# ucsdarclab/Python-SuPer

Measured on AMD Instinct MI355X. Metric: LM iterations/s (embedded-deformation LM, point-to-plane + ARAP + Rot), higher is better.
Workload: dtype f64; 1 GPU; C2: 200000 surfels / 2000 ED nodes / KNN=4, point-to-plane + ARAP + Rot, 10 LM iterations + Surfels.update per frame; frames_per_gpu=8, streams_per_gpu=1, global_frames=8, parallelism=frames sharded over 1 GPU(s), beta all-gather

## Files before the change

include/super_lm.h:

```cpp
#ifndef SUPER_LM_H
#define SUPER_LM_H

#include <stdint.h>

#ifdef __cplusplus
extern "C" {
#endif

enum {
  SLM_OK = 0,
  SLM_ERR_INVALID = 1,
  SLM_ERR_HIP = 2,
  SLM_ERR_NO_DEVICE = 3,
  SLM_ERR_UNBOUND = 4,
  SLM_ERR_UNSUPPORTED = 5
};

enum {
  SLM_ITER_OK = 0,
  SLM_ITER_SOLVER_FAILED = 1,
  SLM_ITER_NOT_RUN = 2,
  SLM_ITER_SOLVER_TIMEOUT = 3
};

// ... 342 lines not shown

typedef struct slm_graph_outputs {
  int32_t cap_nodes, pad;
  double* points;
  double* norms;
  double* radii;
  int32_t* edge_index;
  double* edges_lens;
  int32_t* triangles;
  double* triangles_areas;
} slm_graph_outputs;

int slm_graph_init(int32_t H, int32_t W, int32_t step, const uint8_t* valid, const int32_t* index_map,
                   const double* points, const double* norms, const slm_graph_outputs* out,
                   int32_t* counts_host, void* stream);

int slm_graph_init_semantic(int32_t H, int32_t W, int32_t step, const uint8_t* valid, const int32_t* index_map,
                            const double* points, const double* norms, int32_t num_classes, const double* seg_conf,
                            int32_t prune_class_edges, const slm_graph_outputs* out, int32_t* node_seg,
                            double* node_seg_conf, int32_t* counts_host, void* stream);

int slm_debug_last_solver_form(slm_solver* s);
int slm_debug_last_dag_mode(slm_solver* s);
int slm_debug_counters(int64_t out[4]);
int slm_debug_dag_trace(slm_solver* s, int32_t slot, int32_t on, void* stream);
int slm_debug_dag_timeout(int64_t ticks);
int slm_debug_dag_abort(slm_solver* s, int32_t n_frames, void* stream);
int slm_debug_read(slm_solver* s, int32_t slot, int32_t what, double* host_out, int64_t max_doubles,
                   int64_t* n_doubles, void* stream);
int slm_debug_read_plan(slm_solver* s, int32_t slot, int32_t what, void* host_out, int64_t max_bytes, int64_t* n_bytes,
                        void* stream);

#ifdef __cplusplus
}
#endif
#endif
```

python-super_amd/csrc/slm_api.hip:

```cpp
#include <atomic>
#include <condition_variable>
#include <functional>
#include <mutex>
#include <new>
#include <string>
#include <thread>
#include <algorithm>
#include <vector>
#include <cstdio>
#include <cstring>

#include "slm_common.h"
#include "slm_prep.h"

void launch_data_grad(const FrameDev*, int, int, int, double, hipStream_t);
void launch_data_grad_pairs(const FrameDev*, int, int, int, double, hipStream_t);
void launch_data_loss(const FrameDev*, int, int, int, double, int, hipStream_t);
void launch_data_resid(const FrameDev*, int, int, int, double, double*, uint8_t*, int32_t*, hipStream_t);
void launch_data_gram(const FrameDev*, int, int, double, int, hipStream_t, const int* reuse = nullptr);
void launch_begin_and_gram(const FrameDev*, int, int, double, hipStream_t, const int* reuse, int dag_cut);
void launch_data_eval(const FrameDev*, int, int, double, int mode, hipStream_t, const int* reuse = nullptr);
void launch_band_assemble(const FrameDev*, int, int, hipStream_t);
void launch_reg_grad(const FrameDev*, int, int, int, double, int, double, hipStream_t);
void launch_front_assemble(const FrameDev*, int, int, hipStream_t);
void launch_pair_reduce(const FrameDev*, int, int, hipStream_t);
void launch_pair_scatter(const FrameDev*, int, int, hipStream_t);
void launch_reg_grad_nd(const FrameDev*, int, int, int, double, int, double, hipStream_t);
void launch_front_load_rhs(const FrameDev*, int, int, hipStream_t);
void launch_iter_begin_nd(const FrameDev*, int, hipStream_t, const int* reuse, int dag_cut);
void launch_front_solve(const FrameDev*, int, const NDLevelSched*, int, double, hipStream_t);
int launch_front_solve_dag(const FrameDev*, int, int, double, hipStream_t, int cut, bool reset, bool check);
int dag_device_setup(int dev, int* xcd8_out);
int dag_last_mode();
void launch_after_solve(const FrameDev*, int, int, int, int, double, int, double, int, hipStream_t);
hipError_t set_dag_timeout_ticks(long long);
void launch_dag_abort_check(const FrameDev*, int, hipStream_t);
void launch_front_levels(const FrameDev*, int, const NDLevelSched*, int, int, int, double, hipStream_t);
void launch_reg_loss(const FrameDev*, int, int, int, double, int, double, int, hipStream_t);
void launch_bandwidth(const slm_frame&, int*, hipStream_t);
void launch_band_solve(const FrameDev*, int, int, int, double, hipStream_t);
void launch_band_to_dense(const FrameDev*, int, double*, hipStream_t);
void launch_dense_to_band(const FrameDev*, const double*, const double*, hipStream_t);
void launch_init_slot(const FrameDev*, int, int, const slm_config&, hipStream_t);
void launch_iter_begin(const FrameDev*, int, hipStream_t);
void launch_pack_nodes(const FrameDev*, int, int, hipStream_t);
void launch_make_trial(const FrameDev*, int, int, hipStream_t);
void launch_pack_target(int, const float*, const float*, float4*, hipStream_t);
void launch_pack_target_px(int, const int*, const uint8_t*, const float*, const float*, float4*, hipStream_t);
void launch_accept(const FrameDev*, int, int, int, int, hipStream_t, int* reuse = nullptr, int eval_pass = 0);
void launch_loss_out(const FrameDev*, int, int, double*, hipStream_t);
void launch_zero_reg_part(const FrameDev*, int, int, hipStream_t);
void launch_update(int, int, int, float*, float*, const int*, const float*, float*, float*, const double*,
                   hipStream_t);
void launch_update64(int, int, int, double*, double*, const int*, const double*, double*, double*, const double*,
                     hipStream_t);
void launch_knn(int, int, int, int, const float*, const float*, int*, float*, hipStream_t);
void launch_knn64(int, int, int, int, const double*, const double*, const int*, const int*, int*, double*, int*,
                  hipStream_t);
void launch_knn_weights64(int, int, int, const int*, const double*, const double*, int, const double*, const double*,
                          double*, uint8_t*, hipStream_t);
// ... 220 lines not shown
  std::vector<std::thread> threads_;
  std::mutex m_;
  std::condition_variable cv_work_, cv_done_;
  const std::function<void(int)>* job_ = nullptr;
  int generation_ = 0, n_active_ = 0, pending_ = 0;
  bool stop_ = false;
};
}

struct slm_solver {
  PrepBuffers* prep = nullptr;
  BindPool bind_pool;
  AsyncWorker prep_worker;
  PrepBuffers* prep_async = nullptr;
  hipStream_t prep_stream = nullptr;
  std::vector<PrepBuffers*> bind_prep;
  std::vector<hipStream_t> bind_streams;
  std::vector<hipEvent_t> bind_events;
  std::mutex band_mutex;
  hipEvent_t drain_event = nullptr;
  double drain_est_ms = 0.0;
  int last_solver_form = -1;
  int last_dag_mode = -1;
  bool no_reuse = false;
  bool hybrid_batches = true;
  long dag_max_nodes = 8000;
  bool fuse_begin = true;
  bool pure_fill = true;
  bool profile = false;
  std::vector<hipEvent_t> ev_pool;
  std::vector<std::vector<hipEvent_t>> ev_runs;
  slm_config cfg{};
  std::vector<Slot> slots;
  FrameDev* frames_dev = nullptr;
  int* bw_dev = nullptr;
  int* bw_host = nullptr;
  int* reuse_dev = nullptr;
  int rank = 0, world = 1;
  bool shard_mode = false;
};
namespace {
bool solve_is_task_graph(const slm_solver* s, int n, int J);
}

static std::atomic<long long> g_reallocs{0}, g_realloc_bytes{0}, g_plan_builds{0}, g_plan_reuses{0}, g_plan_fill_hits{0};

// ... 9 lines not shown
  }
  size_t want = need + need / 8;
  hipError_t e = hipMalloc((void**)&p, want * sizeof(T));
  if (e == hipSuccess) cap = want;
  return e;
}
template <typename T>
static hipError_t grow(GP<T>& p, size_t& cap, size_t need) {
  T* q = p;
  const hipError_t e = grow(q, cap, need);
  p = q;
  return e;
}

static int check_slots(slm_solver* s, int first, int n);
static int check_slots_fwd(slm_solver* s, int first, int n) { return check_slots(s, first, n); }

extern "C" {

const char* slm_last_error(void) { return g_err.c_str(); }

int slm_debug_last_solver_form(slm_solver* s) { return s ? s->last_solver_form : -1; }
int slm_debug_last_dag_mode(slm_solver* s) { return s ? s->last_dag_mode : -1; }

int slm_debug_counters(int64_t out[4]) {
  if (!out) return fail(SLM_ERR_INVALID, "slm_debug_counters: null output");
  out[0] = g_reallocs;
  out[1] = g_realloc_bytes;
  out[2] = g_plan_builds;
  out[3] = g_plan_reuses;
  return SLM_OK;
}

int slm_debug_dag_timeout(int64_t ticks) {
  if (ticks < 0) return fail(SLM_ERR_INVALID, "slm_debug_dag_timeout: negative");
  HIPCHK(set_dag_timeout_ticks(ticks == 0 ? 300000000ll : (long long)ticks));
  return SLM_OK;
}

int slm_debug_dag_abort(slm_solver* s, int32_t n_frames, void* stream) {
  int rc = check_slots_fwd(s, 0, n_frames);
  if (rc) return rc;
  for (int i = 0; i < n_frames; ++i)
    if (!s->slots[i].h.nd_ready) return fail(SLM_ERR_UNSUPPORTED, "slm_debug_dag_abort: every slot needs a nested-dissection plan");
  hipStream_t st = (hipStream_t)stream;
  launch_dag_abort_check(s->frames_dev, n_frames, st);
// ... 114 lines not shown
  } catch (...) {
    delete s;
    return fail(SLM_ERR_HIP, "slm_create: out of host memory");
  }
  hipError_t e = hipMalloc((void**)&s->frames_dev, sizeof(FrameDev) * cfg->max_frames);
  if (e == hipSuccess) e = hipMemset(s->frames_dev, 0, sizeof(FrameDev) * cfg->max_frames);
  if (e == hipSuccess) e = hipMalloc((void**)&s->bw_dev, 2 * sizeof(int));
  if (e == hipSuccess) e = hipMalloc((void**)&s->reuse_dev, sizeof(int) * cfg->max_frames);
  if (e == hipSuccess) e = hipMemset(s->reuse_dev, 0, sizeof(int) * cfg->max_frames);
  if (e == hipSuccess) e = hipHostMalloc((void**)&s->bw_host, 2 * sizeof(int), hipHostMallocDefault);
  if (e == hipSuccess) {
    s->prep = prep_create();
    if (!s->prep) e = hipErrorOutOfMemory;
  }
  if (e != hipSuccess) {
    g_err = std::string("slm_create: ") + hipGetErrorString(e);
    slm_destroy(s);
    return SLM_ERR_HIP;
  }
  {
    int dev = 0;
    (void)hipGetDevice(&dev);
    (void)dag_device_setup(dev, nullptr);
  }
  if (const char* hb = getenv("SLM_HYBRID")) s->hybrid_batches = atoi(hb) != 0;
  if (const char* dm = getenv("SLM_DAG_MAX_NODES")) s->dag_max_nodes = atol(dm);
  if (const char* nr = getenv("SLM_NO_REUSE")) s->no_reuse = atoi(nr) != 0;
  if (const char* pf = getenv("SLM_PURE_FILL")) s->pure_fill = atoi(pf) != 0;
  if (const char* fb = getenv("SLM_FUSE_BEGIN")) s->fuse_begin = atoi(fb) != 0;
  *out = s;
  return SLM_OK;
}

int slm_destroy(slm_solver* s) {
  if (!s) return SLM_OK;
  s->prep_worker.shutdown();
  s->bind_pool.shutdown();
  for (Slot& sl : s->slots) {
    FrameDev& h = sl.h;
    if (h.beta) (void)hipFree(h.beta);
    if (h.delta) (void)hipFree(h.delta);
    if (h.rhs) (void)hipFree(h.rhs);
    if (sl.band) (void)hipFree(sl.band);
    if (sl.linv) (void)hipFree(sl.linv);
    if (h.loss_part) (void)hipFree(h.loss_part);
    if (h.st) (void)hipFree(h.st);
    if (h.rec) (void)hipFree(h.rec);
// ... 764 lines not shown
  if (s->cfg.use_arap || s->cfg.use_rot)
    d.n_reg_part = std::min(kRegBlocksMax, (d.maxJKe + 255) / 256);
  return d;
}

static bool solve_is_task_graph(const slm_solver* s, int n, int J) {
  return s->cfg.solver_path == 2 || (s->cfg.solver_path == 0 && (n <= 2 || (long)n * J <= s->dag_max_nodes));
}
static bool solve_is_hybrid(const slm_solver* s, int n, const BatchDims& d) {
  return !solve_is_task_graph(s, n, d.maxP / 7) && (s->cfg.solver_path == 4 || (s->cfg.solver_path == 0 && s->hybrid_batches)) &&
         d.hybrid_cut >= 0 && d.hybrid_levels == (int)d.sched.size() && d.hybrid_cut + 1 < d.hybrid_levels;
}
static int dag_cut_of(const slm_solver* s, int n, const BatchDims& d) {
  if (solve_is_task_graph(s, n, d.maxP / 7)) return -1;
  return solve_is_hybrid(s, n, d) ? d.hybrid_cut : -2;
}
int enqueue_front_solve(slm_solver* s, const FrameDev* fr, int n, const BatchDims& d, double u_override, hipStream_t st,
                        bool dag_reset_done = false, bool dag_check_later = false) {
  const bool dag = solve_is_task_graph(s, n, d.maxP / 7);
  const bool hybrid = solve_is_hybrid(s, n, d);
  s->last_solver_form = dag ? 1 : (hybrid ? 2 : 0);
  int mode = -1;
  if (dag) {
    mode = launch_front_solve_dag(fr, n, d.max_tasks, u_override, st, -1, !dag_reset_done, !dag_check_later);
  } else if (hybrid) {
    const int n_levels = (int)d.sched.size(), l_cut = n_levels - 1 - d.hybrid_cut;
    launch_front_levels(fr, n, d.sched.data(), n_levels, l_cut, 0, u_override, st);
    mode = launch_front_solve_dag(fr, n, d.max_top_tasks, u_override, st, d.hybrid_cut, !dag_reset_done, !dag_check_later);
  } else {
    launch_front_solve(fr, n, d.sched.data(), (int)d.sched.size(), u_override, st);
  }
  s->last_dag_mode = mode;
  return mode;
}

int enqueue_assemble_nd(slm_solver* s, int first, int n, const BatchDims& d, hipStream_t st) {
  const FrameDev* fr = s->frames_dev + first;
  if (s->cfg.use_data && !d.v1 && !d.vk)
    return fail(SLM_ERR_UNSUPPORTED, "slm_solve: a multifrontal slot without a multifrontal data path");
  launch_iter_begin_nd(fr, n, st, nullptr, -2);
  if (s->cfg.use_data) {
    if (d.v1) {
      launch_data_eval(fr, n, kLossBlocks, s->cfg.w_data, 2, st);
      launch_data_gram(fr, n, d.max_pos, s->cfg.w_data, d.gram_variants, st);
      launch_front_assemble(fr, n, d.max_blocks, st);
    } else {
      launch_data_grad_pairs(fr, n, d.maxN, d.K, s->cfg.w_data, st);
      launch_pair_scatter(fr, n, d.max_blocks, st);
    }
  }
  launch_reg_grad_nd(fr, n, d.maxP / 7, s->cfg.use_arap, s->cfg.w_arap, s->cfg.use_rot, s->cfg.w_rot, st);
  if (!s->cfg.use_arap && !s->cfg.use_rot) launch_front_load_rhs(fr, n, d.maxP, st);
  return SLM_OK;
// ... 579 lines not shown
```

python-super_amd/csrc/slm_front.hip:

```cpp
#include <algorithm>
#include <atomic>
#include <cstdlib>

#include "slm_tile.h"
#include "slm_begin.h"

__device__ __forceinline__ int nd_base(const NDFront& f, int p) {
  return p < f.nv ? 7 * p : f.n1p + 7 * (p - f.nv);
}

__device__ __forceinline__ double* ftile(const FrameDev& fd, const NDFront& f, int r, int c) {
  const size_t t = (size_t)c * f.nt - (size_t)c * (c - 1) / 2 + (size_t)(r - c);
  return fd.ftiles + f.tile_off + t * TILE;
}

__device__ __forceinline__ double* front_entry(const FrameDev& fd, const NDFront& f, int i, int j) {
  return ftile(fd, f, i >> 6, j >> 6) + (i & 63) + (size_t)(j & 63) * NB;
}

__device__ __forceinline__ double* dest_entry(const FrameDev& fd, const NDDest& d, int x, int y) {
  const NDFront& f = fd.fronts[d.front];
  const int rb = nd_base(f, d.prow), cb = nd_base(f, d.pcol);
  return d.transpose ? front_entry(fd, f, rb + y, cb + x) : front_entry(fd, f, rb + x, cb + y);
}
// ... 667 lines not shown
    }
    __syncthreads();
    for (int sc = c + 1; sc < f.npt; ++sc) {
      const double* Ls = ftile(fd, f, sc, c);
      double breg[16];
#pragma unroll
      for (int e = 0; e < 16; ++e) breg[e] = Ls[threadIdx.x + 256 * e];
      __syncthreads();
#pragma unroll
      for (int e = 0; e < 16; ++e) Bl[threadIdx.x + 256 * e] = breg[e];
      __syncthreads();
      for (int r = sc; r < f.npt; ++r) {
        double* Ct = ftile(fd, f, r, sc);
        double areg[16];
        load_a_frags(ftile(fd, f, r, c), areg);
        double4_t acc[4];
        load_c_frags(Ct, acc);
        if (r == sc) tile_ABt_regs_trim<true>(areg, Bl, acc, 4, w + 1);
        else tile_ABt_regs<true>(areg, Bl, acc);
        store_c_frags(Ct, acc);
      }
    }
    __syncthreads();
  }
}

__global__ void __launch_bounds__(256, 3) k_fL21(const FrameDev* __restrict__ frames, LevelRef lvl, WgMap map) {
  __shared__ double Bl[TILE];
  __shared__ double yv[NB];
  WgId wg;
  if (!wg_decode(map, wg)) return;
  const FrameDev& fd = frames[wg.frame];
  if (!fd.bound || !fd.nd_ready) return;
  int fi;
  if (!level_front(fd, lvl, wg.front, fi)) return;
  const NDFront& f = fd.fronts[fi];
  const int r = f.npt + wg.unit;
  if (f.npt == 0 || r >= f.nt) return;
  const int w = threadIdx.x >> 6, l = threadIdx.x & 63, lr = l & 15, lk = l >> 4;
  double* vecs = fd.fvec + f.vec_off;
  const bool wave_on = 16 * w < min(NB, 7 * f.nb - NB * wg.unit);
  double rhs_acc = 0.0;
  for (int c = 0; c < f.npt; ++c) {
    {
      const int ncol = min(NB, f.n1 - NB * c);
      const int nblk = (ncol + 15) >> 4;
// ... 334 lines not shown
  hipLaunchKernelGGL(k_pair_scatter, dim3((max_blocks + 3) / 4, n_frames), dim3(256), 0, st, fr);
}

void launch_front_assemble(const FrameDev* fr, int n_frames, int max_blocks, hipStream_t st) {
  if (max_blocks <= 0) return;
  hipLaunchKernelGGL(k_front_assemble, dim3((max_blocks + 3) / 4, n_frames), dim3(256), 0, st, fr);
}

void launch_reg_grad_nd(const FrameDev* fr, int n_frames, int maxJ, int use_arap, double lam_a,
                        int use_rot, double lam_r, hipStream_t st) {
  if (maxJ <= 0 || (!use_arap && !use_rot)) return;
  hipLaunchKernelGGL(k_reg_grad_nd, dim3((maxJ * RG_LANES + 255) / 256, n_frames), dim3(256), 0, st, fr, use_arap,
                     lam_a, use_rot, lam_r);
}

void launch_front_load_rhs(const FrameDev* fr, int n_frames, int maxP, hipStream_t st) {
  hipLaunchKernelGGL(k_front_load_rhs, dim3((maxP + 255) / 256, n_frames), dim3(256), 0, st, fr);
}

void launch_iter_begin_nd(const FrameDev* fr, int n_frames, hipStream_t st, const int* reuse, int dag_cut) {
  hipLaunchKernelGGL(k_iter_begin_nd, dim3(1024, n_frames), dim3(256), 0, st, fr, reuse, dag_cut);
}

void launch_front_levels(const FrameDev* fr, int n_frames, const NDLevelSched* lv, int n_levels, int l_factor_end,
                         int l_back_end, double u_override, hipStream_t st) {
  const size_t lds = PANEL_LDS_DOUBLES * sizeof(double);
  const size_t lds11 = L11_LDS_DOUBLES * sizeof(double);
  static std::atomic<bool> attr_set[64];
  int dev = 0;
  (void)hipGetDevice(&dev);
  const bool tracked = dev >= 0 && dev < 64;
  if (!tracked || !attr_set[dev].load(std::memory_order_acquire)) {
    if (hipFuncSetAttribute((const void*)k_fL11, hipFuncAttributeMaxDynamicSharedMemorySize, (int)lds11) != hipSuccess ||
        hipFuncSetAttribute((const void*)k_fpanel, hipFuncAttributeMaxDynamicSharedMemorySize, (int)lds) != hipSuccess ||
        hipFuncSetAttribute((const void*)k_fpotrf, hipFuncAttributeMaxDynamicSharedMemorySize, (int)lds) != hipSuccess)
      return;
    if (tracked) attr_set[dev].store(true, std::memory_order_release);
  }
  for (int l = 0; l < l_factor_end; ++l) {
    const NDLevelSched& s = lv[l];
    if (s.n_fronts <= 0) continue;
    const LevelRef lr{l, s.first, s.n_fronts};
    static const long compact_min = [] {
      const char* e = getenv("SLM_COMPACT_MIN");
      return e ? atol(e) : 64L;
    }();
    static const int compact_npt = [] {
      const char* e = getenv("SLM_COMPACT_NPT");
      return e ? atoi(e) : 4;
    }();
    const bool compact = s.max_npt <= compact_npt && (long)s.n_fronts * n_frames >= compact_min;
    if (s.n_pull > 0) {
      const int total = s.n_pull * n_frames;
      hipLaunchKernelGGL(k_fpull, dim3((unsigned)((total + 7) / 8 * 8)), dim3(256), 0, st, fr, l, s.n_pull, s.pull_at, n_frames);
    }
    if (compact) {
      hipLaunchKernelGGL(k_fL11, dim3(1, s.n_fronts, n_frames), dim3(256), lds11, st, fr, lr, u_override);
      if (s.max_n2p > 0) {
        const WgMap m = make_map(s.max_n2p / 64, s.n_fronts, n_frames);
        hipLaunchKernelGGL(k_fL21, map_grid(m), dim3(256), 0, st, fr, lr, m);
      }
    }
    for (int c = 0; !compact && c < s.max_npt; ++c) {
      const int mcap = s.max_nt - 1 - c;
      if ((long)(mcap + 1) * s.n_fronts * n_frames <= 512) {
        const WgMap m = make_map(mcap + 1, s.n_fronts, n_frames);
        hipLaunchKernelGGL(k_fpanel, map_grid(m), dim3(256), lds, st, fr, lr, c, u_override, m);
      } else {
        hipLaunchKernelGGL(k_fpotrf, dim3(1, s.n_fronts, n_frames), dim3(256), lds, st, fr, lr, c,
                           u_override);
        if (mcap > 0) {
          const WgMap m = make_map(mcap, s.n_fronts, n_frames);
          hipLaunchKernelGGL(k_ftrsm, map_grid(m), dim3(256), 0, st, fr, lr, c, m);
        }
      }
      const int bcap = std::min(mcap, s.max_npt - 1 - c);
      int ntile = 0;
      for (int b = 1; b <= bcap; ++b) ntile += mcap - b + 1;
      if (ntile + mcap > 0) {
        const WgMap m = make_map(ntile + mcap, s.n_fronts, n_frames);
        hipLaunchKernelGGL(k_ftrail, map_grid(m), dim3(256), 0, st, fr, lr, c, mcap, bcap, ntile, m);
      }
    }
    if (s.n_schur > 0) {
      const int total = s.n_schur * n_frames;
      hipLaunchKernelGGL(k_fschur, dim3((unsigned)((total + 7) / 8 * 8)), dim3(256), 0, st, fr, l, s.n_schur, s.schur_at,
                         n_frames);
    }
  }
  for (int l = l_back_end - 1; l >= 0; --l) {
    const NDLevelSched& s = lv[l];
    if (s.n_fronts <= 0 || s.max_npt <= 0) continue;
    const LevelRef lr{l, s.first, s.n_fronts};
    if (s.max_n2p > 0)
      hipLaunchKernelGGL(k_fback_prep, dim3(s.max_npt, s.n_fronts, n_frames), dim3(256),
                         (size_t)s.max_n2p * sizeof(double), st, fr, lr);
    for (int e = 0; e < s.max_npt; ++e)
      hipLaunchKernelGGL(k_fbacksub, dim3(s.max_npt, s.n_fronts, n_frames), dim3(256), 0, st, fr,
                         lr, e);
  }
}

void launch_front_solve(const FrameDev* fr, int n_frames, const NDLevelSched* lv, int n_levels,
                        double u_override, hipStream_t st) {
  launch_front_levels(fr, n_frames, lv, n_levels, n_levels, 0, u_override, st);
  launch_front_levels(fr, n_frames, lv, n_levels, 0, n_levels, u_override, st);
}
```

python-super_amd/csrc/slm_tile.h:

```cpp
#pragma once
#include "slm_common.h"

typedef double double4_t __attribute__((ext_vector_type(4)));

__device__ __forceinline__ void trace_put(long long* trc, int k, long long v) {
  typedef __attribute__((address_space(1))) long long gll;
  *((gll*)(trc + k)) = v;
}

#define NB SLM_NB
#define TILE (NB * NB)

#define LD NB

__device__ __forceinline__ void wave_sync() {
  __builtin_amdgcn_fence(__ATOMIC_RELEASE, "wavefront");
  __builtin_amdgcn_wave_barrier();
  __builtin_amdgcn_fence(__ATOMIC_ACQUIRE, "wavefront");
}

template <bool NEG>
__device__ __forceinline__ double4_t blk_mma(double4_t acc, const double* X, int xs_m, int xs_p,
                                             const double* Y, int ys_p, int ys_n) {
  const int l = threadIdx.x & 63, lr = l & 15, lk = l >> 4;
// ... 190 lines not shown
  acc = blk_mma<true>(acc, S + ib * 16 + kb * 16 * LD, 1, LD, S + jb * 16 + kb * 16 * LD, LD, 1);
  blk_store(Cb, 1, LD, acc);
}

#define SLM_MAIL_DOUBLES 2560
#define SLM_MAIL_EMPTY 0x7FF8DEADBEEF0001ll
__device__ __forceinline__ void publish_blocks16(const double* S, const double* dinv, int kb, double* g_mail) {
  typedef __attribute__((address_space(1))) double gdbl;
  const int l = threadIdx.x & 63;
#pragma unroll
  for (int j = 0; j < 4; ++j) {
    const int e = l + 64 * j;
    __hip_atomic_store((gdbl*)(g_mail + kb * 256 + e), dinv[kb * 256 + e], __ATOMIC_RELAXED, __HIP_MEMORY_SCOPE_AGENT);
  }
  for (int t = 0; t < kb; ++t)
#pragma unroll
    for (int j = 0; j < 4; ++j) {
      const int e = l + 64 * j, i = e & 15, k = e >> 4;
      __hip_atomic_store((gdbl*)(g_mail + (4 + kb * (kb - 1) / 2 + t) * 256 + e), S[(16 * kb + i) + (16 * t + k) * LD],
                         __ATOMIC_RELAXED, __HIP_MEMORY_SCOPE_AGENT);
    }
}

__device__ __forceinline__ bool factor_inverse64p(double* S, double* M, double* dinv, double* wt, double* xch,
                                                  int* s_ok, int* pf, double* g_mail = nullptr, int* g_early = nullptr,
                                                  long long* trc = nullptr, int nblk = 4, double* la_blk = nullptr,
                                                  const double* la_part = nullptr, double* la_sum = nullptr) {
#define FTRC(k) do { if (trc && threadIdx.x == 0) trace_put(trc, (k), wall_clock64()); } while (0)
  const int w = threadIdx.x >> 6;
  const double4_t z4 = {0.0, 0.0, 0.0, 0.0};
  if (threadIdx.x < 16) pf[threadIdx.x] = 0;
  if (threadIdx.x == 0) *s_ok = 1;
  if (!la_blk) __syncthreads();
  double* Wscr = wt + (w > 0 ? w - 1 : 0) * 256;
  int* vpf = pf;
#pragma unroll 1
  for (int kb = 0; kb < 4; ++kb) {
    FTRC(3 * kb);
    if (w == 0) {
      if (kb < nblk) {
        const bool staged = kb == 0 && la_blk;
        const bool ok = diag16(staged ? la_blk : S + kb * 16 * (LD + 1), dinv + kb * 256, xch, staged ? 16 : LD);
        if (!ok && (threadIdx.x & 63) == 0) *s_ok = 0;
      } else {
        const int l = threadIdx.x & 63;
#pragma unroll
        for (int j = 0; j < 4; ++j) {
          const int e = l + 64 * j;
          dinv[kb * 256 + e] = ((e & 15) == (e >> 4)) ? 1.0 : 0.0;
        }
        wave_sync();
      }
      FTRC(3 * kb + 1);
    } else if (kb == 0) {
      for (int e = threadIdx.x - 64; e < 6 * 256; e += 192) {
        const int b = e >> 8, ib = b < 3 ? 0 : (b < 5 ? 1 : 2), jb = b < 3 ? b + 1 : (b < 5 ? b - 1 : 3);
// ... 15 lines not shown
    } else {
      lds_wait_all(vpf + 8, 1);
      if (w == 3) {
        double4_t t = blk_LM(z4, S + 32 + 16 * LD, dinv + 256, true);
        blk_neg_dinv_store(M + 32 + 16 * LD, dinv + 512, Wscr, t);
        t = blk_LM(z4, S + 48 + 16 * LD, dinv + 256, true);
        t = blk_LM(t, S + 48 + 32 * LD, M + 32 + 16 * LD, false);
        blk_store(Wscr, 1, 16, t);
      } else if (w == 1) {
        double4_t t = blk_LM(z4, S + 32, dinv, true);
        t = blk_LM(t, S + 32 + 16 * LD, M + 16, false);
        blk_neg_dinv_store(M + 32, dinv + 512, Wscr, t);
        t = blk_LM(z4, S + 48, dinv, true);
        t = blk_LM(t, S + 48 + 16 * LD, M + 16, false);
        t = blk_LM(t, S + 48 + 32 * LD, M + 32, false);
        blk_store(Wscr, 1, 16, t);
      } else {
        const double4_t t = blk_LM(z4, S + 48 + 32 * LD, dinv + 512, true);
        blk_store(Wscr, 1, 16, t);
      }
      wave_sync();
    }
    if (kb == 0 && g_early) asm volatile("s_waitcnt vmcnt(0)" ::: "memory");
    __syncthreads();
    FTRC(3 * kb + 2);
    if (kb == 0 && la_part && threadIdx.x < NB)
      *la_sum = la_part[threadIdx.x] + la_part[NB + threadIdx.x] + la_part[2 * NB + threadIdx.x] + la_part[3 * NB + threadIdx.x];
    if (kb == 3) break;
    if (g_mail && w == (kb == 0 ? 3 : 2)) publish_blocks16(S, dinv, kb, g_mail);
    if (kb == 0 && g_early && threadIdx.x == 128)
      __hip_atomic_store((__attribute__((address_space(1))) int*)g_early, 1, __ATOMIC_RELAXED, __HIP_MEMORY_SCOPE_AGENT);
    if (w < 3 - kb) {
      const int ib = kb + 1 + w;
      double* Xb = S + ib * 16 + kb * 16 * LD;
      double4_t acc = blk_mma<false>(z4, Xb, 1, LD, dinv + kb * 256, 16, 1);
      blk_store(Xb, 1, LD, acc);
      wave_sync();
      lds_signal(vpf + 4 * kb + w);
    }
    if (w == 0) {
      blk_trail(S, kb + 1, kb + 1, kb);
      wave_sync();
    }
  }
  if (w >= 1) {
    const int j = (w == 1) ? 0 : (w == 2 ? 2 : 1);
    double4_t m2 = blk_mma<true>(z4, dinv + 768, 1, 16, Wscr, 1, 16);
    blk_store(M + 48 + j * 16 * LD, 1, LD, m2);
  } else {
    if (g_mail) publish_blocks16(S, dinv, 3, g_mail);
    for (int e = threadIdx.x; e < 1024; e += 64) {
      const int b = e >> 8, i = e & 15, k = (e >> 4) & 15;
      M[(16 * b + i) + (16 * b + k) * LD] = dinv[b * 256 + i + 16 * k];
    }
  }
  __syncthreads();
  FTRC(12);
#undef FTRC
  return *s_ok != 0;
}

__device__ __forceinline__ void load_a_frags(const double* __restrict__ A, double areg[16]) {
  const int l = threadIdx.x & 63, w = threadIdx.x >> 6, lr = l & 15, lk = l >> 4;
#pragma unroll
  for (int ks = 0; ks < 16; ++ks) areg[ks] = A[(16 * w + lr) + (size_t)(4 * ks + lk) * NB];
}

__device__ __forceinline__ void load_c_frags(const double* __restrict__ Cg, double4_t acc[4]) {
  const int l = threadIdx.x & 63, w = threadIdx.x >> 6, lr = l & 15, lk = l >> 4;
#pragma unroll
  for (int ni = 0; ni < 4; ++ni)
#pragma unroll
    for (int r = 0; r < 4; ++r) acc[ni][r] = Cg[(16 * w + lr) + (size_t)(16 * ni + lk + 4 * r) * NB];
}

template <bool NEGATE, bool LOWER_B = false>
__device__ __forceinline__ void tile_ABt_regs(const double areg[16], const double* Bl,
                                              double4_t acc[4]) {
  const int l = threadIdx.x & 63, lr = l & 15, lk = l >> 4;
// ... 77 lines not shown
```

python-super_amd/super_amd/_lib.py:

```python
from __future__ import annotations

import ctypes as C
import os

_PKG_ROOT = os.path.dirname(os.path.dirname(os.path.abspath(__file__)))
LIB_PATH = os.path.join(_PKG_ROOT, "lib", os.environ.get("SLM_LIB", "libsuper_lm.so"))

SLM_OK = 0
SLM_ERR_INVALID, SLM_ERR_HIP, SLM_ERR_NO_DEVICE, SLM_ERR_UNBOUND, SLM_ERR_UNSUPPORTED = 1, 2, 3, 4, 5
SLM_ITER_OK, SLM_ITER_SOLVER_FAILED, SLM_ITER_NOT_RUN, SLM_ITER_SOLVER_TIMEOUT = 0, 1, 2, 3
SLM_ABI_VERSION = 3
PLAN_INFO_DOUBLES = 14
SLM_X_PAIR_BLOCKS, SLM_X_DELTA, SLM_X_DATA_LOSS = 0, 1, 2
PHASES = ["zero", "data_grad", "reg_grad", "solve", "data_loss", "accept"]

GF_NTERMS = 10

EXPORTS = [
    "slm_create", "slm_destroy", "slm_last_error", "slm_device_count", "slm_bind_frame", "slm_bind_frames",
    "slm_run", "slm_profile_enable", "slm_profile_read", "slm_get_plan_info", "slm_get_beta", "slm_set_beta", "slm_get_records", "slm_assemble", "slm_loss",
    "slm_solve", "slm_solve_dense", "slm_data_residuals", "slm_apply_update", "slm_knn",
    "slm_knn_weights", "slm_gf_create", "slm_gf_destroy", "slm_gf_bind_frame", "slm_gf_run",
    "slm_gf_bind_semantic", "slm_gf_bind_flow", "slm_gf_get_edge_points", "slm_gf_set_shard", "slm_gf_eval_morph",
    "slm_gf_eval_losses", "slm_gf_step", "slm_gf_get_partial", "slm_gf_set_partial",
    "slm_depth_create", "slm_depth_destroy", "slm_depth_preprocess",
    "slm_graph_init", "slm_fuse_create", "slm_fuse_destroy", "slm_fuse_input_data", "slm_fuse_swap_stable",
    "slm_fuse_bind_semantic", "slm_knn_f64", "slm_knn_weights_f64", "slm_graph_init_semantic", "slm_debug_counters", "slm_debug_last_solver_form", "slm_debug_last_dag_mode",
    "slm_set_shard", "slm_lm_grad_local", "slm_lm_solve", "slm_lm_loss_local", "slm_lm_accept",
    "slm_lm_exchange_size", "slm_lm_exchange_get", "slm_lm_exchange_set", "slm_lm_exchange_ptr",
    "slm_gf_get_deform", "slm_gf_loss_grad", "slm_apply_update_gf",
    "slm_apply_update_f64", "slm_apply_update_gf_f64", "slm_debug_read", "slm_debug_dag_trace",
    "slm_abi_version", "slm_abi_check", "slm_debug_dag_timeout", "slm_debug_dag_abort", "slm_prepare_model", "slm_discard_prepared", "slm_debug_read_plan",
    "slm_render_create", "slm_render_destroy", "slm_render_points", "slm_gf_render",
    "slm_render_backward", "slm_render_ssim_loss", "slm_gf_bind_point_grad",
]


class SlmConfig(C.Structure):
    _fields_ = [("num_iterations", C.c_int32), ("phase_test", C.c_int32), ("use_data", C.c_int32),
                ("use_arap", C.c_int32), ("use_rot", C.c_int32), ("max_frames", C.c_int32),
                ("data_path", C.c_int32), ("solver_path", C.c_int32),
                ("w_data", C.c_double), ("w_arap", C.c_double), ("w_rot", C.c_double),
                ("u0", C.c_double), ("v", C.c_double), ("minimal_loss0", C.c_double)]


class SlmFrame(C.Structure):
    _fields_ = [("N", C.c_int32), ("J", C.c_int32), ("T", C.c_int32), ("H", C.c_int32),
                ("W", C.c_int32), ("K", C.c_int32), ("K_ED", C.c_int32),
                ("fx", C.c_float), ("fy", C.c_float), ("cx", C.c_float), ("cy", C.c_float),
                ("sf_points", C.c_void_p), ("sf_knn_idx", C.c_void_p), ("sf_knn_w", C.c_void_p),
# ... 107 lines not shown
def load():
    global _lib
    if _lib is not None:
        return _lib
    import torch
    if not os.path.exists(LIB_PATH):
        raise SuperLMError(
            f"{LIB_PATH} not found: build it with `python python-super_amd/super_amd/build.py` "
            "(hipcc, gfx950). There is no CPU fallback.")
    lib = C.CDLL(LIB_PATH)
    vp, i32, dbl = C.c_void_p, C.c_int32, C.c_double
    lib.slm_last_error.restype = C.c_char_p
    lib.slm_last_error.argtypes = []
    lib.slm_device_count.restype = C.c_int
    lib.slm_device_count.argtypes = []
    sig = {
        "slm_create": [C.POINTER(SlmConfig), C.POINTER(vp)],
        "slm_destroy": [vp],
        "slm_debug_counters": [C.POINTER(C.c_int64)],
        "slm_debug_read": [vp, i32, i32, vp, C.c_int64, C.POINTER(C.c_int64), vp],
        "slm_debug_dag_trace": [vp, i32, i32, vp],
        "slm_debug_last_solver_form": [vp],
        "slm_debug_last_dag_mode": [vp],
        "slm_bind_frames": [vp, i32, i32, C.POINTER(SlmFrame), vp],
        "slm_bind_frame": [vp, i32, C.POINTER(SlmFrame), vp],
        "slm_prepare_model": [vp, i32, C.POINTER(SlmFrame), vp],
        "slm_discard_prepared": [vp, i32],
        "slm_debug_read_plan": [vp, i32, i32, vp, C.c_int64, C.POINTER(C.c_int64), vp],
        "slm_run": [vp, i32, vp],
        "slm_profile_enable": [vp, i32],
        "slm_get_plan_info": [vp, i32, C.POINTER(C.c_double), i32],
        "slm_abi_check": [i32, i32, i32, i32, i32, i32],
        "slm_debug_dag_timeout": [C.c_int64],
        "slm_debug_dag_abort": [vp, i32, vp],
        "slm_profile_read": [vp, C.POINTER(C.c_double), C.POINTER(C.c_int64)],
        "slm_get_beta": [vp, i32, vp, vp],
        "slm_set_beta": [vp, i32, vp, vp],
        "slm_get_records": [vp, i32, C.POINTER(SlmIterRecord), i32, vp],
        "slm_assemble": [vp, i32, vp, vp, vp],
        "slm_loss": [vp, i32, vp, vp],
        "slm_solve": [vp, i32, dbl, vp, vp, vp],
        "slm_solve_dense": [i32, vp, vp, vp, vp, vp],
        "slm_data_residuals": [vp, i32, vp, vp, vp, vp],
        "slm_apply_update": [i32, i32, i32, vp, vp, vp, vp, vp, vp, vp, vp],
        "slm_knn": [i32, i32, i32, i32, vp, vp, vp, vp, vp],
        "slm_knn_weights": [i32, i32, i32, vp, vp, vp, vp, vp, vp],
# ... 68 lines not shown
```

Before: 3344 LM it/s.

## Add warp-specialized chained L11 front factor kernel for small front levels

Adds a 512-thread k_fchain kernel that, for compact levels with few fronts and at most four panel tiles, splits the workgroup into two wave groups. One group factors and inverts diagonal tiles while the other applies the trailing Schur updates and RHS eliminations, synchronised by an LDS counter barrier. It replaces k_fL11 when fronts×frames fits within the CU count, aiming to overlap the diagonal factorisation with the panel updates. The cost is more complex synchronisation and a spin barrier that could hang or slow down if misused.

New measurement: 3388 LM it/s, median of 6. 1.3% higher.

```diff
diff --git a/include/super_lm.h b/include/super_lm.h
--- a/include/super_lm.h
+++ b/include/super_lm.h
@@ -388,6 +388,7 @@
 
 int slm_debug_last_solver_form(slm_solver* s);
 int slm_debug_last_dag_mode(slm_solver* s);
+int slm_debug_last_chain_levels(slm_solver* s);
 int slm_debug_counters(int64_t out[4]);
 int slm_debug_dag_trace(slm_solver* s, int32_t slot, int32_t on, void* stream);
 int slm_debug_dag_timeout(int64_t ticks);
diff --git a/python-super_amd/csrc/slm_api.hip b/python-super_amd/csrc/slm_api.hip
--- a/python-super_amd/csrc/slm_api.hip
+++ b/python-super_amd/csrc/slm_api.hip
@@ -28,14 +28,14 @@
 void launch_reg_grad_nd(const FrameDev*, int, int, int, double, int, double, hipStream_t);
 void launch_front_load_rhs(const FrameDev*, int, int, hipStream_t);
 void launch_iter_begin_nd(const FrameDev*, int, hipStream_t, const int* reuse, int dag_cut);
-void launch_front_solve(const FrameDev*, int, const NDLevelSched*, int, double, hipStream_t);
+int launch_front_solve(const FrameDev*, int, const NDLevelSched*, int, double, hipStream_t, long);
 int launch_front_solve_dag(const FrameDev*, int, int, double, hipStream_t, int cut, bool reset, bool check);
 int dag_device_setup(int dev, int* xcd8_out);
 int dag_last_mode();
 void launch_after_solve(const FrameDev*, int, int, int, int, double, int, double, int, hipStream_t);
 hipError_t set_dag_timeout_ticks(long long);
 void launch_dag_abort_check(const FrameDev*, int, hipStream_t);
-void launch_front_levels(const FrameDev*, int, const NDLevelSched*, int, int, int, double, hipStream_t);
+int launch_front_levels(const FrameDev*, int, const NDLevelSched*, int, int, int, double, hipStream_t, long);
 void launch_reg_loss(const FrameDev*, int, int, int, double, int, double, int, hipStream_t);
 void launch_bandwidth(const slm_frame&, int*, hipStream_t);
 void launch_band_solve(const FrameDev*, int, int, int, double, hipStream_t);
@@ -302,6 +302,8 @@
   double drain_est_ms = 0.0;
   int last_solver_form = -1;
   int last_dag_mode = -1;
+  int last_chain_levels = -1;
+  long chain_max = 0;
   bool no_reuse = false;
   bool hybrid_batches = true;
   long dag_max_nodes = 8000;
@@ -357,6 +359,7 @@
 
 int slm_debug_last_solver_form(slm_solver* s) { return s ? s->last_solver_form : -1; }
 int slm_debug_last_dag_mode(slm_solver* s) { return s ? s->last_dag_mode : -1; }
+int slm_debug_last_chain_levels(slm_solver* s) { return s ? s->last_chain_levels : -1; }
 
 int slm_debug_counters(int64_t out[4]) {
   if (!out) return fail(SLM_ERR_INVALID, "slm_debug_counters: null output");
@@ -517,7 +520,10 @@
     int dev = 0;
     (void)hipGetDevice(&dev);
     (void)dag_device_setup(dev, nullptr);
-  }
+    int n_cu = 0;
+    if (hipDeviceGetAttribute(&n_cu, hipDeviceAttributeMultiprocessorCount, dev) == hipSuccess) s->chain_max = n_cu;
+  }
+  if (const char* ch = getenv("SLM_CHAIN")) s->chain_max = atol(ch);
   if (const char* hb = getenv("SLM_HYBRID")) s->hybrid_batches = atoi(hb) != 0;
   if (const char* dm = getenv("SLM_DAG_MAX_NODES")) s->dag_max_nodes = atol(dm);
   if (const char* nr = getenv("SLM_NO_REUSE")) s->no_reuse = atoi(nr) != 0;
@@ -1328,13 +1334,14 @@
   s->last_solver_form = dag ? 1 : (hybrid ? 2 : 0);
   int mode = -1;
   if (dag) {
+    s->last_chain_levels = 0;
     mode = launch_front_solve_dag(fr, n, d.max_tasks, u_override, st, -1, !dag_reset_done, !dag_check_later);
   } else if (hybrid) {
     const int n_levels = (int)d.sched.size(), l_cut = n_levels - 1 - d.hybrid_cut;
-    launch_front_levels(fr, n, d.sched.data(), n_levels, l_cut, 0, u_override, st);
+    s->last_chain_levels = launch_front_levels(fr, n, d.sched.data(), n_levels, l_cut, 0, u_override, st, s->chain_max);
     mode = launch_front_solve_dag(fr, n, d.max_top_tasks, u_override, st, d.hybrid_cut, !dag_reset_done, !dag_check_later);
   } else {
-    launch_front_solve(fr, n, d.sched.data(), (int)d.sched.size(), u_override, st);
+    s->last_chain_levels = launch_front_solve(fr, n, d.sched.data(), (int)d.sched.size(), u_override, st, s->chain_max);
   }
   s->last_dag_mode = mode;
   return mode;
diff --git a/python-super_amd/csrc/slm_front.hip b/python-super_amd/csrc/slm_front.hip
--- a/python-super_amd/csrc/slm_front.hip
+++ b/python-super_amd/csrc/slm_front.hip
@@ -713,6 +713,232 @@
       }
     }
     __syncthreads();
+  }
+}
+
+#define CHAIN_LDS_DOUBLES (4 * TILE + 7 * 256 + 2 * NB + 5 * NB + 16)
+#define CHAIN_THREADS 512
+#define CHAIN_MAX_NPT 4
+
+__device__ __forceinline__ void ch_load(const double* __restrict__ T, double4_t x[4], int w, int l) {
+  const int lr = l & 15, lk = l >> 4;
+#pragma unroll
+  for (int ni = 0; ni < 4; ++ni)
+#pragma unroll
+    for (int r = 0; r < 4; ++r) x[ni][r] = T[(16 * w + lr) + (size_t)(16 * ni + lk + 4 * r) * NB];
+}
+__device__ __forceinline__ void ch_store(double* __restrict__ T, const double4_t x[4], int w, int l) {
+  const int lr = l & 15, lk = l >> 4;
+#pragma unroll
+  for (int ni = 0; ni < 4; ++ni)
+#pragma unroll
+    for (int r = 0; r < 4; ++r) T[(16 * w + lr) + (size_t)(16 * ni + lk + 4 * r) * NB] = x[ni][r];
+}
+__device__ __forceinline__ void ch_areg(const double4_t x[4], double a[16]) {
+#pragma unroll
+  for (int ni = 0; ni < 4; ++ni)
+#pragma unroll
+    for (int r = 0; r < 4; ++r) a[4 * ni + r] = x[ni][r];
+}
+__device__ __forceinline__ void ch_rhs(const double4_t L[4], const double* yv, double* rhs_r, int w, int l) {
+  const int lr = l & 15, lk = l >> 4;
+  double sacc = 0.0;
+#pragma unroll
+  for (int ni = 0; ni < 4; ++ni)
+#pragma unroll
+    for (int rr = 0; rr < 4; ++rr) sacc += L[ni][rr] * yv[16 * ni + lk + 4 * rr];
+  sacc += __shfl_xor(sacc, 16, 64);
+  sacc += __shfl_xor(sacc, 32, 64);
+  if (lk == 0) rhs_r[16 * w + lr] -= sacc;
+}
+
+__device__ __forceinline__ int ch_tid() {
+  int t = threadIdx.x;
+  asm volatile("" : "+v"(t));
+  return t;
+}
+__device__ __forceinline__ int ch_lane() { return ch_tid() & 63; }
+__device__ __forceinline__ void ch_enter(double* S, int c, int n1, double u) {
+  const int t0 = ch_tid();
+#pragma unroll
+  for (int t = 0; t < 16; ++t) {
+    const int e = t0 + 256 * t;
+    const int i = e % NB, k = e / NB;
+    double x = (i >= k) ? S[e] : 0.0;
+    if (i == k) x = (c * NB + i < n1) ? x + u : 1.0;
+    S[e] = x;
+  }
+}
+
+__global__ void __launch_bounds__(CHAIN_THREADS, 1) k_fchain(const FrameDev* __restrict__ frames, LevelRef lvl,
+                                                             double u_override) {
+  extern __shared__ double lds[];
+  double* S = lds;
+  double* M = lds + TILE;
+  double* Bl = lds + 2 * TILE;
+  double* Mb = lds + 3 * TILE;
+  double* dinv = lds + 4 * TILE;
+  double* wt = dinv + 4 * 256;
+  double* vec = wt + 3 * 256;
+  double* rhs = vec + 2 * NB;
+  double* yv = rhs + 4 * NB;
+  int* s_ok = reinterpret_cast<int*>(yv + NB);
+  int* pf = s_ok + 8;
+  int* bar = pf + 16;
+  const FrameDev& fd = frames[blockIdx.z];
+  if (!fd.bound || !fd.nd_ready) return;
+  int fi;
+  if (!level_front(fd, lvl, blockIdx.y, fi)) return;
+  const NDFront& f = fd.fronts[fi];
+  const int npt = f.npt;
+  if (npt == 0) return;
+  const double u = (u_override >= 0.0) ? u_override : fd.st->u;
+  double* vecs = fd.fvec + f.vec_off;
+  const int wv = __builtin_amdgcn_readfirstlane(threadIdx.x >> 6);
+  const bool grp_a = wv < 4;
+  const int w = wv & 3;
+  const LdsGroupBarrier bar_a{bar, 4}, bar_b{bar + 1, 4};
+
+  if (threadIdx.x < 2) bar[threadIdx.x] = 0;
+  for (int e = threadIdx.x; e < npt * NB; e += CHAIN_THREADS) rhs[e] = vecs[e];
+  if (grp_a) {
+    const double* src = ftile(fd, f, 0, 0);
+#pragma unroll
+    for (int t = 0; t < 16; ++t) S[threadIdx.x + 256 * t] = src[threadIdx.x + 256 * t];
+  }
+  __syncthreads();
+
+  if (grp_a) {
+    for (int s = 0; s < npt; ++s) {
+      ch_enter(S, s, f.n1, u);
+      const bool ok = factor_inverse64p(S, M, dinv, wt, vec, s_ok, pf, nullptr, nullptr, nullptr,
+                                        min(4, (f.n1 - s * NB + 15) >> 4), nullptr, nullptr, nullptr, bar_a);
+      if (!ok && threadIdx.x == 0) fd.st->chol_fail = 1;
+      __syncthreads();
+      double* linv = fd.flinv + f.linv_off + (size_t)s * TILE;
+      const int t0 = ch_tid();
+      for (int e = t0; e < TILE; e += 256) {
+        const double m = M[e];
+        linv[e] = m;
+        Mb[e] = m;
+      }
+      if (t0 < NB) {
+        const int i = t0;
+        const double* rs = rhs + (size_t)s * NB;
+        double acc = 0.0;
+        for (int k = 0; k <= i; ++k) acc += M[i + k * LD] * rs[k];
+        yv[i] = acc;
+        vecs[(size_t)s * NB + i] = acc;
+      }
+      __syncthreads();
+      __syncthreads();
+    }
+  } else {
+    double4_t xn[4], cn[4];
+    {
+      const int l = ch_lane();
+      if (npt > 1) {
+        ch_load(ftile(fd, f, 1, 0), xn, w, l);
+        ch_load(ftile(fd, f, 1, 1), cn, w, l);
+      }
+    }
+    for (int s = 0; s < npt; ++s) {
+      if (s > 0) {
+        const int c = s - 1;
+        const int l = ch_lane();
+        {
+          double4_t lsc[4];
+          ch_load(Bl, lsc, w, l);
+          ch_rhs(lsc, yv, rhs + (size_t)s * NB, w, l);
+        }
+        if (s + 1 < npt) {
+          double4_t Lr[2][4];
+#pragma unroll
+          for (int j = 0; j < 2; ++j) {
+            const int r = s + 1 + j;
+            if (r < npt) {
+              double4_t a4[4];
+              ch_load(ftile(fd, f, r, c), a4, w, l);
+              double areg[16];
+              ch_areg(a4, areg);
+#pragma unroll
+              for (int ni = 0; ni < 4; ++ni) Lr[j][ni] = double4_t{0.0, 0.0, 0.0, 0.0};
+              tile_ABt_regs<false, true>(areg, Mb, Lr[j]);
+              ch_store(ftile(fd, f, r, c), Lr[j], w, l);
+              ch_rhs(Lr[j], yv, rhs + (size_t)r * NB, w, l);
+              __builtin_amdgcn_sched_barrier(0);
+            }
+          }
+#pragma unroll
+          for (int j = 0; j < 2; ++j) {
+            const int r = s + 1 + j;
+            if (r < npt) {
+              double4_t acc[4];
+              ch_load(ftile(fd, f, r, s), acc, w, l);
+              double areg[16];
+              ch_areg(Lr[j], areg);
+              tile_ABt_regs<true>(areg, Bl, acc);
+              if (j == 0) {
+#pragma unroll
+                for (int ni = 0; ni < 4; ++ni) xn[ni] = acc[ni];
+              } else {
+                ch_store(ftile(fd, f, r, s), acc, w, l);
+              }
+              __builtin_amdgcn_sched_barrier(0);
+            }
+          }
+#pragma unroll
+          for (int jq = 0; jq < 2; ++jq) {
+            const int q = s + 1 + jq;
+            if (q < npt) {
+              bar_b();
+              ch_store(Bl, Lr[jq], w, l);
+              bar_b();
+#pragma unroll
+              for (int j = jq; j < 2; ++j) {
+                const int r = s + 1 + j;
+                if (r < npt) {
+                  double4_t acc[4];
+                  ch_load(ftile(fd, f, r, q), acc, w, l);
+                  double areg[16];
+                  ch_areg(Lr[j], areg);
+                  if (r == q) tile_ABt_regs_trim<true>(areg, Bl, acc, 4, w + 1);
+                  else tile_ABt_regs<true>(areg, Bl, acc);
+                  if (j == 0) {
+#pragma unroll
+                    for (int ni = 0; ni < 4; ++ni) cn[ni] = acc[ni];
+                  } else {
+                    ch_store(ftile(fd, f, r, q), acc, w, l);
+                  }
+                  __builtin_amdgcn_sched_barrier(0);
+                }
+              }
+            }
+          }
+        }
+      }
+      __syncthreads();
+      if (s + 1 < npt) {
+        const int l = ch_lane();
+        double areg[16];
+        ch_areg(xn, areg);
+#pragma unroll
+        for (int ni = 0; ni < 4; ++ni) xn[ni] = double4_t{0.0, 0.0, 0.0, 0.0};
+        tile_ABt_regs<false, true>(areg, M, xn);
+        ch_store(ftile(fd, f, s + 1, s), xn, w, l);
+        ch_store(Bl, xn, w, l);
+      }
+      __syncthreads();
+      if (s + 1 < npt) {
+        const int l = ch_lane();
+        double areg[16];
+        ch_areg(xn, areg);
+        tile_ABt_regs_trim<true>(areg, Bl, cn, 4, w + 1);
+        ch_store(ftile(fd, f, s + 1, s + 1), cn, w, l);
+        ch_store(S, cn, w, l);
+      }
+      __syncthreads();
+    }
   }
 }
 
@@ -1093,19 +1319,22 @@
   hipLaunchKernelGGL(k_iter_begin_nd, dim3(1024, n_frames), dim3(256), 0, st, fr, reuse, dag_cut);
 }
 
-void launch_front_levels(const FrameDev* fr, int n_frames, const NDLevelSched* lv, int n_levels, int l_factor_end,
-                         int l_back_end, double u_override, hipStream_t st) {
+int launch_front_levels(const FrameDev* fr, int n_frames, const NDLevelSched* lv, int n_levels, int l_factor_end,
+                        int l_back_end, double u_override, hipStream_t st, long chain_max) {
   const size_t lds = PANEL_LDS_DOUBLES * sizeof(double);
   const size_t lds11 = L11_LDS_DOUBLES * sizeof(double);
+  const size_t lds_chain = CHAIN_LDS_DOUBLES * sizeof(double);
+  int n_chain = 0;
   static std::atomic<bool> attr_set[64];
   int dev = 0;
   (void)hipGetDevice(&dev);
   const bool tracked = dev >= 0 && dev < 64;
   if (!tracked || !attr_set[dev].load(std::memory_order_acquire)) {
     if (hipFuncSetAttribute((const void*)k_fL11, hipFuncAttributeMaxDynamicSharedMemorySize, (int)lds11) != hipSuccess ||
+        hipFuncSetAttribute((const void*)k_fchain, hipFuncAttributeMaxDynamicSharedMemorySize, (int)lds_chain) != hipSuccess ||
         hipFuncSetAttribute((const void*)k_fpanel, hipFuncAttributeMaxDynamicSharedMemorySize, (int)lds) != hipSuccess ||
         hipFuncSetAttribute((const void*)k_fpotrf, hipFuncAttributeMaxDynamicSharedMemorySize, (int)lds) != hipSuccess)
-      return;
+      return 0;
     if (tracked) attr_set[dev].store(true, std::memory_order_release);
   }
   for (int l = 0; l < l_factor_end; ++l) {
@@ -1126,7 +1355,12 @@
       hipLaunchKernelGGL(k_fpull, dim3((unsigned)((total + 7) / 8 * 8)), dim3(256), 0, st, fr, l, s.n_pull, s.pull_at, n_frames);
     }
     if (compact) {
-      hipLaunchKernelGGL(k_fL11, dim3(1, s.n_fronts, n_frames), dim3(256), lds11, st, fr, lr, u_override);
+      if ((long)s.n_fronts * n_frames <= chain_max && s.max_npt <= CHAIN_MAX_NPT) {
+        hipLaunchKernelGGL(k_fchain, dim3(1, s.n_fronts, n_frames), dim3(CHAIN_THREADS), lds_chain, st, fr, lr, u_override);
+        ++n_chain;
+      } else {
+        hipLaunchKernelGGL(k_fL11, dim3(1, s.n_fronts, n_frames), dim3(256), lds11, st, fr, lr, u_override);
+      }
       if (s.max_n2p > 0) {
         const WgMap m = make_map(s.max_n2p / 64, s.n_fronts, n_frames);
         hipLaunchKernelGGL(k_fL21, map_grid(m), dim3(256), 0, st, fr, lr, m);
@@ -1170,10 +1404,12 @@
       hipLaunchKernelGGL(k_fbacksub, dim3(s.max_npt, s.n_fronts, n_frames), dim3(256), 0, st, fr,
                          lr, e);
   }
-}
-
-void launch_front_solve(const FrameDev* fr, int n_frames, const NDLevelSched* lv, int n_levels,
-                        double u_override, hipStream_t st) {
-  launch_front_levels(fr, n_frames, lv, n_levels, n_levels, 0, u_override, st);
-  launch_front_levels(fr, n_frames, lv, n_levels, 0, n_levels, u_override, st);
-}
+  return n_chain;
+}
+
+int launch_front_solve(const FrameDev* fr, int n_frames, const NDLevelSched* lv, int n_levels,
+                       double u_override, hipStream_t st, long chain_max) {
+  const int n_chain = launch_front_levels(fr, n_frames, lv, n_levels, n_levels, 0, u_override, st, chain_max);
+  launch_front_levels(fr, n_frames, lv, n_levels, 0, n_levels, u_override, st, chain_max);
+  return n_chain;
+}
diff --git a/python-super_amd/csrc/slm_tile.h b/python-super_amd/csrc/slm_tile.h
--- a/python-super_amd/csrc/slm_tile.h
+++ b/python-super_amd/csrc/slm_tile.h
@@ -236,16 +236,37 @@
     }
 }
 
+struct WgBarrier {
+  __device__ __forceinline__ void operator()() const { __syncthreads(); }
+};
+struct LdsGroupBarrier {
+  int* cnt;
+  int n;
+  __device__ __forceinline__ void operator()() const {
+    __builtin_amdgcn_fence(__ATOMIC_RELEASE, "workgroup");
+    if ((threadIdx.x & 63) == 0) {
+      const int old = __hip_atomic_fetch_add(cnt, 1, __ATOMIC_RELAXED, __HIP_MEMORY_SCOPE_WORKGROUP);
+      const int target = (old / n + 1) * n;
+      for (int it = 0; it < (1 << 23) && __hip_atomic_load(cnt, __ATOMIC_RELAXED, __HIP_MEMORY_SCOPE_WORKGROUP) < target; ++it)
+        __builtin_amdgcn_s_sleep(1);
+    }
+    __builtin_amdgcn_wave_barrier();
+    __builtin_amdgcn_fence(__ATOMIC_ACQUIRE, "workgroup");
+  }
+};
+
+template <class Bar = WgBarrier>
 __device__ __forceinline__ bool factor_inverse64p(double* S, double* M, double* dinv, double* wt, double* xch,
                                                   int* s_ok, int* pf, double* g_mail = nullptr, int* g_early = nullptr,
                                                   long long* trc = nullptr, int nblk = 4, double* la_blk = nullptr,
-                                                  const double* la_part = nullptr, double* la_sum = nullptr) {
+                                                  const double* la_part = nullptr, double* la_sum = nullptr,
+                                                  const Bar bar = Bar()) {
 #define FTRC(k) do { if (trc && threadIdx.x == 0) trace_put(trc, (k), wall_clock64()); } while (0)
   const int w = threadIdx.x >> 6;
   const double4_t z4 = {0.0, 0.0, 0.0, 0.0};
   if (threadIdx.x < 16) pf[threadIdx.x] = 0;
   if (threadIdx.x == 0) *s_ok = 1;
-  if (!la_blk) __syncthreads();
+  if (!la_blk) bar();
   double* Wscr = wt + (w > 0 ? w - 1 : 0) * 256;
   int* vpf = pf;
 #pragma unroll 1
@@ -307,7 +328,7 @@
       wave_sync();
     }
     if (kb == 0 && g_early) asm volatile("s_waitcnt vmcnt(0)" ::: "memory");
-    __syncthreads();
+    bar();
     FTRC(3 * kb + 2);
     if (kb == 0 && la_part && threadIdx.x < NB)
       *la_sum = la_part[threadIdx.x] + la_part[NB + threadIdx.x] + la_part[2 * NB + threadIdx.x] + la_part[3 * NB + threadIdx.x];
@@ -339,7 +360,7 @@
       M[(16 * b + i) + (16 * b + k) * LD] = dinv[b * 256 + i + 16 * k];
     }
   }
-  __syncthreads();
+  bar();
   FTRC(12);
 #undef FTRC
   return *s_ok != 0;
diff --git a/python-super_amd/super_amd/_lib.py b/python-super_amd/super_amd/_lib.py
--- a/python-super_amd/super_amd/_lib.py
+++ b/python-super_amd/super_amd/_lib.py
@@ -25,7 +25,7 @@
     "slm_gf_eval_losses", "slm_gf_step", "slm_gf_get_partial", "slm_gf_set_partial",
     "slm_depth_create", "slm_depth_destroy", "slm_depth_preprocess",
     "slm_graph_init", "slm_fuse_create", "slm_fuse_destroy", "slm_fuse_input_data", "slm_fuse_swap_stable",
-    "slm_fuse_bind_semantic", "slm_knn_f64", "slm_knn_weights_f64", "slm_graph_init_semantic", "slm_debug_counters", "slm_debug_last_solver_form", "slm_debug_last_dag_mode",
+    "slm_fuse_bind_semantic", "slm_knn_f64", "slm_knn_weights_f64", "slm_graph_init_semantic", "slm_debug_counters", "slm_debug_last_solver_form", "slm_debug_last_dag_mode", "slm_debug_last_chain_levels",
     "slm_set_shard", "slm_lm_grad_local", "slm_lm_solve", "slm_lm_loss_local", "slm_lm_accept",
     "slm_lm_exchange_size", "slm_lm_exchange_get", "slm_lm_exchange_set", "slm_lm_exchange_ptr",
     "slm_gf_get_deform", "slm_gf_loss_grad", "slm_apply_update_gf",
@@ -179,6 +179,7 @@
         "slm_debug_dag_trace": [vp, i32, i32, vp],
         "slm_debug_last_solver_form": [vp],
         "slm_debug_last_dag_mode": [vp],
+        "slm_debug_last_chain_levels": [vp],
         "slm_bind_frames": [vp, i32, i32, C.POINTER(SlmFrame), vp],
         "slm_bind_frame": [vp, i32, C.POINTER(SlmFrame), vp],
         "slm_prepare_model": [vp, i32, C.POINTER(SlmFrame), vp],
```
